# alibaba/easydist

Measured on AMD Instinct MI355X. Metric: gpt2_train_samples_per_sec, higher is better.
Workload: dtype bf16; 1 GPU; model=gpt2-small, global_batch=64, seq_len=1024, parallelism=auto(dp1)

## Files before the change

### easydist_amd/ops/csrc/gemm_kernels.hip

```cpp
#include "common.h"
#include "attn_block_map.h"
#include "gemm_tn_map.h"
#include <torch/extension.h>
#include <ATen/cuda/CUDAContext.h>

using f32x4 = __attribute__((ext_vector_type(4))) float;
using bf16x8v = __attribute__((ext_vector_type(8))) __bf16;
using v4s = __attribute__((ext_vector_type(4))) short;
using v8s = __attribute__((ext_vector_type(8))) short;

DEVINL void glds16(const void* gsrc, void* lds_dst) {
  __builtin_amdgcn_global_load_lds(
      (const __attribute__((address_space(1))) unsigned int*)gsrc,
      (__attribute__((address_space(3))) unsigned int*)lds_dst, 16, 0, 0);
}

DEVINL void raw_barrier() { __builtin_amdgcn_s_barrier(); }

#define GELU_C 0.7978845608028654f
#define GELU_A 0.044715f

DEVINL float fast_tanh(float u) {
  return 1.f - 2.f / (__expf(2.f * u) + 1.f);
}

DEVINL float act_apply(int act, float x, float aux) {
  if (act == 1 || act == 3) {
    float u = GELU_C * (x + GELU_A * x * x * x);
    return 0.5f * x * (1.f + fast_tanh(u));
  }
  if (act == 2 || act == 4) {
    float u = GELU_C * (aux + GELU_A * aux * aux * aux);
    float t = fast_tanh(u);
    float d = 0.5f * (1.f + t)
              + 0.5f * aux * (1.f - t * t) * GELU_C
                    * (1.f + 3.f * GELU_A * aux * aux);
    return x * d;
  }
  if (act >= 5) {
    float u = GELU_C * (x + GELU_A * x * x * x);
    return 0.5f * x * (1.f + fast_tanh(u));
  }
  return x;
}

__global__ void __launch_bounds__(256)
gelu_fwd_kernel(const bf16* __restrict__ X, bf16* __restrict__ Y, long n) {
  long i = ((long)blockIdx.x * blockDim.x + threadIdx.x) * 8;
  for (; i + 7 < n; i += (long)gridDim.x * blockDim.x * 8) {
    bf16x8v x = *reinterpret_cast<const bf16x8v*>(&X[i]);
    bf16x8v y;
    #pragma unroll
    for (int e = 0; e < 8; ++e)
      y[e] = (__bf16)act_apply(1, bf2f((bf16)x[e]), 0.f);
    *reinterpret_cast<bf16x8v*>(&Y[i]) = y;
  }
}

__global__ void __launch_bounds__(256)
gelu_bwd_kernel(const bf16* __restrict__ G, const bf16* __restrict__ X,
                bf16* __restrict__ Y, long n) {
  long i = ((long)blockIdx.x * blockDim.x + threadIdx.x) * 8;
  for (; i + 7 < n; i += (long)gridDim.x * blockDim.x * 8) {
    bf16x8v g = *reinterpret_cast<const bf16x8v*>(&G[i]);
    bf16x8v x = *reinterpret_cast<const bf16x8v*>(&X[i]);
    bf16x8v y;
    #pragma unroll
    for (int e = 0; e < 8; ++e)
      y[e] = (__bf16)act_apply(2, bf2f((bf16)g[e]), bf2f((bf16)x[e]));
    *reinterpret_cast<bf16x8v*>(&Y[i]) = y;
  }
}

#define BM 128
#define BN 128
#define BK 32

extern "C" __global__ void __launch_bounds__(256)
gemm_nt_128(const bf16* __restrict__ A, const bf16* __restrict__ Bt,
            bf16* __restrict__ C, const bf16* __restrict__ bias,
            int M, int N, int K) {
  extern __shared__ __attribute__((aligned(16))) char smem[];
  const unsigned ATILE = BM * BK * 2;
  const unsigned BUF = 2 * ATILE;

  unsigned nwg_m = (M + BM - 1) / BM, nwg_n = (N + BN - 1) / BN;
  unsigned wg = xcd_swizzle(blockIdx.x, nwg_m * nwg_n);
  const unsigned m0 = (wg / nwg_n) * BM;
  const unsigned n0 = (wg % nwg_n) * BN;

  const int t = threadIdx.x;
  const int lane = t % WAVE;
  const int wave = t / WAVE;
  const int wm = (wave / 2) * 64;
  const int wn = (wave % 2) * 64;

  auto stage = [&](int buf, int k0) {
    #pragma unroll
    for (int p = 0; p < 2; ++p) {
      int e = (t + p * 256) * 8;
      int row = e / BK, col = e % BK;
      int grow = min((int)m0 + row, M - 1);
      const bf16* src = A + (long)grow * K + k0 + col;
      glds16(src, smem + buf * BUF + (p * 256 + wave * 64) * 16);
    }
    #pragma unroll
    for (int p = 0; p < 2; ++p) {
      int e = (t + p * 256) * 8;
      int row = e / BK, col = e % BK;
      int grow = min((int)n0 + row, N - 1);
      const bf16* src = Bt + (long)grow * K + k0 + col;
      glds16(src, smem + buf * BUF + ATILE + (p * 256 + wave * 64) * 16);
    }
  };

  f32x4 acc[4][4];
  #pragma unroll
  for (int i = 0; i < 4; ++i)
    #pragma unroll
    for (int j = 0; j < 4; ++j)
      acc[i][j] = {0.f, 0.f, 0.f, 0.f};

  stage(0, 0);
  __builtin_amdgcn_s_waitcnt(0);
  __syncthreads();

  const int frag_row = lane & 15;
  const int frag_k = (lane >> 4) * 8;

  int nk = K / BK;
  for (int kt = 0; kt < nk; ++kt) {
    int buf = kt & 1;
    if (kt + 1 < nk) stage(buf ^ 1, (kt + 1) * BK);
    bf16x8v a_frag[4], b_frag[4];
    const char* base = smem;
    #pragma unroll
    for (int i = 0; i < 4; ++i) {
      unsigned off = buf * BUF + ((wm + i * 16 + frag_row) * BK + frag_k) * 2;
      a_frag[i] = *reinterpret_cast<const bf16x8v*>(base + off);
    }
    #pragma unroll
    for (int j = 0; j < 4; ++j) {
      unsigned off = buf * BUF + ATILE +
                     ((wn + j * 16 + frag_row) * BK + frag_k) * 2;
      b_frag[j] = *reinterpret_cast<const bf16x8v*>(base + off);
    }
    #pragma unroll
    for (int i = 0; i < 4; ++i)
      #pragma unroll
      for (int j = 0; j < 4; ++j)
        acc[i][j] = __builtin_amdgcn_mfma_f32_16x16x32_bf16(
            a_frag[i], b_frag[j], acc[i][j], 0, 0, 0);
    __builtin_amdgcn_s_waitcnt(0);
    __syncthreads();
  }

  const int c_col = lane & 15;
  const int c_row0 = (lane >> 4) * 4;
  float bias_v[4] = {0.f, 0.f, 0.f, 0.f};
  if (bias) {
    #pragma unroll
    for (int j = 0; j < 4; ++j)
      bias_v[j] = bf2f(bias[min((int)(n0 + wn + j * 16 + c_col), N - 1)]);
  }
  #pragma unroll
  for (int i = 0; i < 4; ++i) {
    #pragma unroll
    for (int j = 0; j < 4; ++j) {
      #pragma unroll
      for (int reg = 0; reg < 4; ++reg) {
        int gm = m0 + wm + i * 16 + c_row0 + reg;
        int gn = n0 + wn + j * 16 + c_col;
        if (gm < M && gn < N)
          C[(long)gm * N + gn] = f2bf(acc[i][j][reg] + bias_v[j]);
      }
    }
  }
}

#define BM2 256
#define BN2 256
#define BK2 64
#define HALF_B 16384u
#define BUF_B 65536u

DEVINL unsigned sw32(unsigned x) { return x ^ (((x >> 8) & 7u) << 4); }

extern "C" __global__ void __launch_bounds__(512)
gemm_nt_256(const bf16* __restrict__ A, const bf16* __restrict__ Bt,
            bf16* __restrict__ C, const bf16* __restrict__ bias,
            bf16* __restrict__ aux, int act, int M, int N, int K) {
  extern __shared__ __attribute__((aligned(16))) char smem[];

  unsigned nwg_m = (M + BM2 - 1) / BM2, nwg_n = (N + BN2 - 1) / BN2;
  unsigned wg = xcd_swizzle(blockIdx.x, nwg_m * nwg_n);
  const unsigned m0 = (wg / nwg_n) * BM2;
  const unsigned n0 = (wg % nwg_n) * BN2;

  const int t = threadIdx.x;
  const int lane = t % WAVE;
  const int wave = t / WAVE;
  const int wr = wave >> 2;
  const int wc = wave & 3;

  auto stage_a = [&](int parity, int k0, int h) {
    unsigned dst0 = parity * BUF_B + h * HALF_B;
    #pragma unroll
    for (int i = 0; i < 2; ++i) {
      unsigned p = (i * 512 + t) * 16;
      unsigned L = sw32(p);
      int s = L >> 13;
      int row = (L >> 7) & 63;
      int k = (L & 127) >> 1;
      int grow = min((int)m0 + s * 128 + h * 64 + row, M - 1);
      glds16(A + (long)grow * K + k0 + k,
             smem + dst0 + (i * 512 + wave * 64) * 16);
    }
  };
  auto stage_b = [&](int parity, int k0, int h) {
    unsigned dst0 = parity * BUF_B + 32768u + h * HALF_B;
    #pragma unroll
    for (int i = 0; i < 2; ++i) {
      unsigned p = (i * 512 + t) * 16;
      unsigned L = sw32(p);
      int s = (L >> 12) & 3;
      int col = (L >> 7) & 31;
      int k = (L & 127) >> 1;
      int gcol = min((int)n0 + s * 64 + h * 32 + col, N - 1);
      glds16(Bt + (long)gcol * K + k0 + k,
             smem + dst0 + (i * 512 + wave * 64) * 16);
    }
  };

  const int fr = lane & 15;
  const int fg = lane >> 4;
  auto read_a = [&](bf16x8v (&a)[4][2], int tile, int mh) {
    unsigned base = (tile & 1) * BUF_B + mh * HALF_B;
    #pragma unroll
    for (int i = 0; i < 4; ++i)
      #pragma unroll
      for (int kk = 0; kk < 2; ++kk) {
        unsigned L = wr * 8192u + (i * 16 + fr) * 128u +
                     (kk * 32 + fg * 8) * 2u;
        a[i][kk] = *reinterpret_cast<const bf16x8v*>(smem + base + sw32(L));
      }
  };
  auto read_b = [&](bf16x8v (&b)[2][2], int tile, int nh) {
    unsigned base = (tile & 1) * BUF_B + 32768u + nh * HALF_B;
    #pragma unroll
    for (int j = 0; j < 2; ++j)
      #pragma unroll
      for (int kk = 0; kk < 2; ++kk) {
        unsigned L = wc * 4096u + (j * 16 + fr) * 128u +
                     (kk * 32 + fg * 8) * 2u;
        b[j][kk] = *reinterpret_cast<const bf16x8v*>(smem + base + sw32(L));
      }
  };

  f32x4 acc[8][4];
  #pragma unroll
  for (int i = 0; i < 8; ++i)
    #pragma unroll
    for (int j = 0; j < 4; ++j)
      acc[i][j] = {0.f, 0.f, 0.f, 0.f};

  bf16x8v a_frag[4][2], b_frag[2][2], b0_frag[2][2];
  const int NT = K / BK2;

  auto k_of = [&](int t) { return t < NT ? t * BK2 : 0; };

  stage_a(0, 0, 0); stage_a(0, 0, 1); stage_b(0, 0, 0); stage_b(0, 0, 1);
  stage_a(1, k_of(1), 0); stage_b(1, k_of(1), 1); stage_a(1, k_of(1), 1);
  asm volatile("s_waitcnt vmcnt(6)" ::: "memory");
  raw_barrier();

  auto mfma_quad = [&](int mh, int nh, bf16x8v (&bf)[2][2]) {
    __builtin_amdgcn_s_setprio(1);
    #pragma unroll
    for (int i = 0; i < 4; ++i)
      #pragma unroll
      for (int j = 0; j < 2; ++j)
        #pragma unroll
        for (int kk = 0; kk < 2; ++kk)
          acc[mh * 4 + i][nh * 2 + j] = __builtin_amdgcn_mfma_f32_16x16x32_bf16(
              a_frag[i][kk], bf[j][kk], acc[mh * 4 + i][nh * 2 + j],
              0, 0, 0);
    __builtin_amdgcn_s_setprio(0);
  };

  for (int T = 0; T < NT; ++T) {
    read_a(a_frag, T, 0);
    read_b(b0_frag, T, 0);
    read_b(b_frag, T, 1);
    stage_b((T + 1) & 1, k_of(T + 1), 0);
    mfma_quad(0, 0, b0_frag);
    raw_barrier();
    stage_a(T & 1, k_of(T + 2), 0);
    mfma_quad(0, 1, b_frag);
    raw_barrier();
    read_a(a_frag, T, 1);
    stage_b(T & 1, k_of(T + 2), 1);
    mfma_quad(1, 1, b_frag);
    raw_barrier();
    stage_a(T & 1, k_of(T + 2), 1);
    asm volatile("s_waitcnt vmcnt(6)" ::: "memory");
    mfma_quad(1, 0, b0_frag);
    raw_barrier();
  }

  asm volatile("s_waitcnt vmcnt(0)" ::: "memory");
  raw_barrier();
  bf16* share = reinterpret_cast<bf16*>(smem) + wave * 8192;
  const unsigned wm = wr * 128, wn = wc * 64;
  float bias_v[4] = {0.f, 0.f, 0.f, 0.f};
  if (bias) {
    #pragma unroll
    for (int j = 0; j < 4; ++j)
      bias_v[j] = bf2f(bias[min((int)(n0 + wn + j * 16 + fr), N - 1)]);
  }
  #pragma unroll
  for (int i = 0; i < 8; ++i)
    #pragma unroll
    for (int j = 0; j < 4; ++j)
      #pragma unroll
      for (int r = 0; r < 4; ++r) {
        int row = i * 16 + fg * 4 + r;
        int col = j * 16 + fr;
        share[row * 64 + col] = f2bf(acc[i][j][r] + bias_v[j]);
      }
  lds_fence();
  #pragma unroll
  for (int tt = 0; tt < 16; ++tt) {
    int row = tt * 8 + (lane >> 3);
    int colc = (lane & 7) * 8;
    int gm = m0 + wm + row;
    int gn = n0 + wn + colc;
    if (gm < (int)M && gn + 8 <= (int)N) {
      bf16x8v val = *reinterpret_cast<const bf16x8v*>(&share[row * 64 + colc]);
      if (act) {
        bf16x8v av{};
        if (act == 2 || act == 4)
          av = *reinterpret_cast<const bf16x8v*>(&aux[(long)gm * N + gn]);
        else if (act >= 5)
          *reinterpret_cast<bf16x8v*>(&aux[(long)gm * N + gn]) = val;
        #pragma unroll
        for (int e = 0; e < 8; ++e)
          val[e] = (__bf16)act_apply(act, bf2f((bf16)val[e]),
                                     bf2f((bf16)av[e]));
      }
      *reinterpret_cast<bf16x8v*>(&C[(long)gm * N + gn]) = val;
    } else if (gm < (int)M) {
      for (int e = 0; e < 8 && gn + e < (int)N; ++e) {
        float xv = bf2f(share[row * 64 + colc + e]);
        float axv = (act == 2 || act == 4)
                        ? bf2f(aux[(long)gm * N + gn + e]) : 0.f;
        if (act >= 5) aux[(long)gm * N + gn + e] = f2bf(xv);
        C[(long)gm * N + gn + e] = f2bf(act_apply(act, xv, axv));
      }
    }
  }
}

#define TBR 32
#define TBP 128
#define TBP2 256

constexpr unsigned tn_img_bytes(int tile) { return TBR * tile * 2; }
constexpr unsigned tn_lds_bytes(int tile, int ring) {
  return (ring ? 3 : 2) * 2 * tn_img_bytes(tile);
}

DEVINL int tn_unswz(int pos) { return ((pos >> 2) & 1) | ((pos & 3) << 1); }

template <int NTHR>
DEVINL void tn_stage(const bf16* src, long ld, int r0, int p0, int pmax,
                     char* dst_base, int t, int wave) {
  #pragma unroll
  for (int i = 0; i < 2; ++i) {
    unsigned p = (i * NTHR + t) * 16;
    int chunk16 = p >> 10;
    unsigned w = p & 1023u;
    int bpos = w >> 7;
    int blk = tn_unswz(bpos);
    int rr = blk * 4 + ((w & 127) >> 5);
    int pp = chunk16 * 16 + ((w & 31) >> 1);
    int gp = min(p0 + pp, pmax - 8);
    glds16(src + (long)(r0 + rr) * ld + gp,
           dst_base + (i * NTHR + wave * 64) * 16);
  }
}

DEVINL bf16x8v tn_frag(const char* img, int chunk, int lane) {
  const char* base = img + chunk * 1024 + (lane >> 4) * 128 + (lane & 15) * 8;
  v4s lo = __builtin_amdgcn_ds_read_tr16_b64_v4i16(
      (__attribute__((address_space(3))) v4s*)base);
  v4s hi = __builtin_amdgcn_ds_read_tr16_b64_v4i16(
      (__attribute__((address_space(3))) v4s*)(base + 512));
  v8s out = __builtin_shufflevector(lo, hi, 0, 1, 2, 3, 4, 5, 6, 7);
  return __builtin_bit_cast(bf16x8v, out);
}

template <int TILE, int RING>
DEVINL void tn_body(const bf16* __restrict__ Ag, const bf16* __restrict__ Bg,
                    float* __restrict__ Cw, float* __restrict__ Asum, int R,
                    int P, int Q, int splitr, int map_mode) {
  extern __shared__ __attribute__((aligned(16))) char smem[];
  constexpr int NTHR = 2 * TILE;
  constexpr int NJ = TILE / 32;
  const unsigned IMG = tn_img_bytes(TILE);
  const unsigned BUF = 2 * IMG;

  unsigned nwg_p = (P + TILE - 1) / TILE, nwg_q = (Q + TILE - 1) / TILE;
  unsigned ntile = nwg_p * nwg_q;
  const TnBlock blk = gemm_tn_map(blockIdx.x, ntile, splitr, map_mode);
  const unsigned tile = blk.tile, slice = blk.slice;
  const unsigned p0 = (tile / nwg_q) * TILE;
  const unsigned q0 = (tile % nwg_q) * TILE;

  int nrt_all = R / TBR;
  int per = (nrt_all + splitr - 1) / splitr;
  int rt0 = slice * per;
  int rt1 = min(nrt_all, rt0 + per);
  if (rt0 >= rt1) return;

  const int t = threadIdx.x;
  const int lane = t % WAVE;
  const int wave = t / WAVE;
  const int wp = (wave >> 1) * 64;
  const int wq = (wave & 1) * (TILE / 2);

  auto stage = [&](int buf, int rt) {
    if (rt < rt1) {
      tn_stage<NTHR>(Ag, P, rt * TBR, p0, P, smem + buf * BUF, t, wave);
      tn_stage<NTHR>(Bg, Q, rt * TBR, q0, Q, smem + buf * BUF + IMG, t, wave);
    }
  };

  f32x4 acc[4][NJ];
  float asum_acc[4] = {0.f, 0.f, 0.f, 0.f};
  #pragma unroll
  for (int i = 0; i < 4; ++i)
    #pragma unroll
    for (int j = 0; j < NJ; ++j)
      acc[i][j] = {0.f, 0.f, 0.f, 0.f};

  auto compute = [&](const char* img) {
    bf16x8v a_frag[4], b_frag[NJ];
    #pragma unroll
    for (int i = 0; i < 4; ++i)
      a_frag[i] = tn_frag(img, (wp >> 4) + i, lane);
    if (Asum && q0 == 0 && (wave & 1) == 0) {
      #pragma unroll
      for (int i = 0; i < 4; ++i) {
        float acc_s = 0.f;
        #pragma unroll
        for (int u = 0; u < 8; ++u) acc_s += bf2f((bf16)a_frag[i][u]);
        asum_acc[i] += acc_s;
      }
    }
    #pragma unroll
    for (int j = 0; j < NJ; ++j)
      b_frag[j] = tn_frag(img + IMG, (wq >> 4) + j, lane);
    #pragma unroll
    for (int i = 0; i < 4; ++i)
      #pragma unroll
      for (int j = 0; j < NJ; ++j)
        acc[i][j] = __builtin_amdgcn_mfma_f32_16x16x32_bf16(
            a_frag[i], b_frag[j], acc[i][j], 0, 0, 0);
  };

  if constexpr (RING) {
    stage(0, rt0);
    stage(1, rt0 + 1);
    int buf = 0;
    for (int rt = rt0; rt < rt1; ++rt) {
      if (rt + 1 < rt1)
        asm volatile("s_waitcnt vmcnt(4)" ::: "memory");
      else
        asm volatile("s_waitcnt vmcnt(0)" ::: "memory");
      raw_barrier();
      stage(buf == 0 ? 2 : buf - 1, rt + 2);
      compute(smem + buf * BUF);
      buf = buf == 2 ? 0 : buf + 1;
    }
  } else {
    stage(0, rt0);
    __builtin_amdgcn_s_waitcnt(0);
    __syncthreads();
    for (int rt = rt0; rt < rt1; ++rt) {
      int buf = (rt - rt0) & 1;
      stage(buf ^ 1, rt + 1);
      compute(smem + buf * BUF);
      __builtin_amdgcn_s_waitcnt(0);
      __syncthreads();
    }
  }

  if (Asum && q0 == 0 && (wave & 1) == 0) {
    #pragma unroll
    for (int i = 0; i < 4; ++i) {
      float v = asum_acc[i];
      v += __shfl_down(v, 32, WAVE);
      v += __shfl_down(v, 16, WAVE);
      if (lane < 16) {
        int gp = p0 + wp + i * 16 + lane;
        if (gp < P) atomicAdd(&Asum[gp], v);
      }
    }
  }
  const int c_col = lane & 15;
  const int c_row0 = (lane >> 4) * 4;
  #pragma unroll
  for (int i = 0; i < 4; ++i)
    #pragma unroll
    for (int j = 0; j < NJ; ++j)
      #pragma unroll
      for (int reg = 0; reg < 4; ++reg) {
        int gp = p0 + wp + i * 16 + c_row0 + reg;
        int gq = q0 + wq + j * 16 + c_col;
        if (gp < P && gq < Q) {
          if (splitr == 1)
            Cw[(long)gp * Q + gq] = acc[i][j][reg];
          else
            atomicAdd(&Cw[(long)gp * Q + gq], acc[i][j][reg]);
        }
      }
}

#define TN_KERNEL(name, tile, ring)                                         \
  extern "C" __global__ void __launch_bounds__(2 * tile)                    \
  name(const bf16* __restrict__ Ag, const bf16* __restrict__ Bg,            \
       float* __restrict__ Cw, float* __restrict__ Asum, int R, int P,      \
       int Q, int splitr, int map_mode) {                                   \
    tn_body<tile, ring>(Ag, Bg, Cw, Asum, R, P, Q, splitr, map_mode);       \
  }
TN_KERNEL(gemm_tn_kernel, TBP, 0)
TN_KERNEL(gemm_tn_256_kernel, TBP2, 1)
TN_KERNEL(gemm_tn_256_drain_kernel, TBP2, 0)


at::Tensor gemm_nt_act(const at::Tensor& a, const at::Tensor& bt,
                       const std::optional<at::Tensor>& bias, int64_t act,
                       const std::optional<at::Tensor>& aux) {
  TORCH_CHECK(a.dtype() == at::kBFloat16 && bt.dtype() == at::kBFloat16);
  TORCH_CHECK(a.is_contiguous() && bt.is_contiguous(),
              "gemm_nt wants K-contiguous operands");
  const long M = a.size(0), K = a.size(1), N = bt.size(0);
  TORCH_CHECK(bt.size(1) == K);
  TORCH_CHECK(K % BK == 0, "gemm_nt: K must be a multiple of 32");
  TORCH_CHECK(N % 8 == 0, "gemm_nt: N must be a multiple of 8");
  auto c = at::empty({M, N}, a.options());
  auto stream = at::cuda::getCurrentCUDAStream();
  const bf16* bias_p = bias ? (const bf16*)bias->data_ptr() : nullptr;
  TORCH_CHECK(!(act == 2 || act >= 4) || aux,
              "gemm_nt: activation modes 2/4/5/6 need aux");
  if (K % BK2 == 0 && M >= BM2 && N >= 128) {
    unsigned nwg = ((M + BM2 - 1) / BM2) * ((N + BN2 - 1) / BN2);
    bf16* aux_p = aux ? (bf16*)aux->data_ptr() : nullptr;
    hipLaunchKernelGGL(gemm_nt_256, dim3(nwg), dim3(512), 2 * BUF_B, stream,
        (const bf16*)a.data_ptr(), (const bf16*)bt.data_ptr(),
        (bf16*)c.data_ptr(), bias_p, aux_p, (int)act, (int)M, (int)N,
        (int)K);
  } else {
    unsigned nwg = ((M + BM - 1) / BM) * ((N + BN - 1) / BN);
    size_t lds = 2 * 2 * BM * BK * 2;
    hipLaunchKernelGGL(gemm_nt_128, dim3(nwg), dim3(256), lds, stream,
        (const bf16*)a.data_ptr(), (const bf16*)bt.data_ptr(),
        (bf16*)c.data_ptr(), bias_p, (int)M, (int)N, (int)K);
    if (act) {
      if (act == 1) c = at::gelu(c, "tanh");
      else if (act == 3) c = at::gelu(c);
      else if (act == 2) c = at::gelu_backward(c, aux.value(), "tanh");
      else if (act == 4) c = at::gelu_backward(c, aux.value(), "none");
      else if (act >= 5) {
        aux.value().copy_(c);
        c = at::gelu(c, "tanh");
      }
    }
  }
  return c;
}

at::Tensor gemm_nt(const at::Tensor& a, const at::Tensor& bt,
                   const std::optional<at::Tensor>& bias) {
  return gemm_nt_act(a, bt, bias, 0, std::nullopt);
}

at::Tensor gelu_fast(const at::Tensor& x) {
  TORCH_CHECK(x.dtype() == at::kBFloat16 && x.is_contiguous());
  const long n = x.numel();
  TORCH_CHECK(n % 8 == 0, "gelu_fast: numel multiple of 8");
  auto y = at::empty_like(x);
  long thr = n / 8;
  unsigned grid = (unsigned)std::min<long>((thr + 255) / 256, 8192);
  auto stream = at::cuda::getCurrentCUDAStream();
  hipLaunchKernelGGL(gelu_fwd_kernel, dim3(grid), dim3(256), 0, stream,
                     (const bf16*)x.data_ptr(), (bf16*)y.data_ptr(), n);
  return y;
}

at::Tensor gelu_bwd_fast(const at::Tensor& g, const at::Tensor& x) {
  TORCH_CHECK(g.dtype() == at::kBFloat16 && g.is_contiguous());
  TORCH_CHECK(x.dtype() == at::kBFloat16 && x.is_contiguous());
  const long n = x.numel();
  TORCH_CHECK(g.numel() == n && n % 8 == 0);
  auto y = at::empty_like(x);
  long thr = n / 8;
  unsigned grid = (unsigned)std::min<long>((thr + 255) / 256, 8192);
  auto stream = at::cuda::getCurrentCUDAStream();
  hipLaunchKernelGGL(gelu_bwd_kernel, dim3(grid), dim3(256), 0, stream,
                     (const bf16*)g.data_ptr(), (const bf16*)x.data_ptr(),
                     (bf16*)y.data_ptr(), n);
  return y;
}

std::tuple<at::Tensor, at::Tensor>
gemm_nt_gelu(const at::Tensor& a, const at::Tensor& bt,
             const std::optional<at::Tensor>& bias, bool tanh_approx) {
  const long M = a.size(0), K = a.size(1), N = bt.size(0);
  if (K % BK2 == 0 && M >= BM2 && N >= 128) {
    auto pre = at::empty({M, N}, a.options());
    auto act = gemm_nt_act(a, bt, bias, tanh_approx ? 5 : 6, pre);
    return {act, pre};
  }
  auto pre = gemm_nt_act(a, bt, bias, 0, std::nullopt);
  auto act = at::gelu(pre, tanh_approx ? "tanh" : "none");
  return {act, pre};
}

std::tuple<at::Tensor, at::Tensor> gemm_tn_asum(const at::Tensor& a,
                                                const at::Tensor& b);

static inline int ed_tn_map_mode() {
  const char* e = getenv("EASYDIST_TN_MAP");
  return (e && atoi(e) == 0) ? TN_MAP_TILE_MAJOR : TN_MAP_SLICE_MAJOR;
}

static at::Tensor tn_launch(const at::Tensor& a, const at::Tensor& b,
                            float* asum_p) {
  const int map_mode = ed_tn_map_mode();
  TORCH_CHECK(a.dtype() == at::kBFloat16 && b.dtype() == at::kBFloat16);
  TORCH_CHECK(a.is_contiguous() && b.is_contiguous());
  const long R = a.size(0), P = a.size(1), Q = b.size(0) == R ? b.size(1) : -1;
  TORCH_CHECK(Q > 0, "gemm_tn: reduce dims must match");
  TORCH_CHECK(R % TBR == 0, "gemm_tn: R must be a multiple of 32");
  TORCH_CHECK(P % TBP == 0 && Q % TBP == 0,
              "gemm_tn: P, Q must be multiples of 128");
  bool big = R / TBR >= 64 && P >= TBP2 && Q >= TBP2;
  unsigned ntile;
  int splitr = 1;
  if (big) {
    ntile = ((P + TBP2 - 1) / TBP2) * ((Q + TBP2 - 1) / TBP2);
    const int target = 256;
    splitr = std::max(1, target / (int)ntile);
    if (const char* e = getenv("EASYDIST_TN256_SPLITR"))
      if (atoi(e) > 0) splitr = atoi(e);
    splitr = std::min((long)splitr, R / TBR / 8);
    splitr = std::max(1, std::min(splitr, 64));
  } else {
    ntile = (P / TBP) * (Q / TBP);
    while (ntile * splitr < 512 && splitr < 16 &&
           (R / TBR) % (splitr * 2) == 0 && (R / TBR) / (splitr * 2) >= 1)
      splitr *= 2;
  }
  auto cw = splitr == 1
      ? at::empty({P, Q}, a.options().dtype(at::kFloat))
      : at::zeros({P, Q}, a.options().dtype(at::kFloat));
  auto stream = at::cuda::getCurrentCUDAStream();
  if (big) {
    const char* se = getenv("EASYDIST_TN256_STAGING");
    const bool ring = !(se && atoi(se) == 0);
    auto kern = ring ? gemm_tn_256_kernel : gemm_tn_256_drain_kernel;
    size_t lds = tn_lds_bytes(TBP2, ring);
    hipLaunchKernelGGL(kern, dim3(ntile * splitr), dim3(2 * TBP2),
        lds, stream,
        (const bf16*)a.data_ptr(), (const bf16*)b.data_ptr(),
        cw.data_ptr<float>(), asum_p, (int)R, (int)P, (int)Q, splitr,
        map_mode);
  } else {
    size_t lds = tn_lds_bytes(TBP, 0);
    hipLaunchKernelGGL(gemm_tn_kernel, dim3(ntile * splitr), dim3(2 * TBP),
        lds, stream,
        (const bf16*)a.data_ptr(), (const bf16*)b.data_ptr(),
        cw.data_ptr<float>(), asum_p, (int)R, (int)P, (int)Q, splitr,
        map_mode);
  }
  return cw;
}

at::Tensor gemm_tn(const at::Tensor& a, const at::Tensor& b) {
  return tn_launch(a, b, nullptr).to(at::kBFloat16);
}

std::tuple<at::Tensor, at::Tensor> gemm_tn_asum(const at::Tensor& a,
                                                const at::Tensor& b) {
  auto asum = at::zeros({a.size(1)}, a.options().dtype(at::kFloat));
  auto cw = tn_launch(a, b, asum.data_ptr<float>());
  return {cw.to(at::kBFloat16), asum};
}
```

Before: 794.9 samples/sec.

## Fuse split-R TN GEMM epilogue with persistent workspace and bf16 sweep

Reworks how the weight-gradient TN GEMM finishes. By default it keeps a persistent per-stream fp32 workspace that the split-R kernel accumulates into atomically. A small sweep kernel then converts it to bf16, copies out the bias sum and re-zeroes the workspace, replacing the per-call zeros allocation and separate .to(bf16) cast. A store mode with per-slice slabs and a last-arriving-block reduction is also added, and single-slice cases now write bf16 directly through an LDS bounce. This adds workspace state keyed by stream and counter logic, and falls back to the old path during graph capture.

```diff
diff --git a/easydist_amd/ops/csrc/gemm_kernels.hip b/easydist_amd/ops/csrc/gemm_kernels.hip
--- a/easydist_amd/ops/csrc/gemm_kernels.hip
+++ b/easydist_amd/ops/csrc/gemm_kernels.hip
@@ -3,6 +3,9 @@
 #include "gemm_tn_map.h"
 #include <torch/extension.h>
 #include <ATen/cuda/CUDAContext.h>
+#include <map>
+#include <mutex>
+#include <type_traits>
 
 using f32x4 = __attribute__((ext_vector_type(4))) float;
 using bf16x8v = __attribute__((ext_vector_type(8))) __bf16;
@@ -366,8 +369,13 @@
 #define TBP2 256
 
 constexpr unsigned tn_img_bytes(int tile) { return TBR * tile * 2; }
+constexpr int tn_bounce_ld(int tile) { return tile / 2 + 4; }
+constexpr unsigned tn_bounce_bytes(int tile) {
+  return (tile / 32) * 16 * tn_bounce_ld(tile) * 4;
+}
 constexpr unsigned tn_lds_bytes(int tile, int ring) {
-  return (ring ? 3 : 2) * 2 * tn_img_bytes(tile);
+  unsigned stage = (ring ? 3 : 2) * 2 * tn_img_bytes(tile);
+  return stage > tn_bounce_bytes(tile) ? stage : tn_bounce_bytes(tile);
 }
 
 DEVINL int tn_unswz(int pos) { return ((pos >> 2) & 1) | ((pos & 3) << 1); }
@@ -390,6 +398,12 @@
   }
 }
 
+#define TN_FIN_LEGACY 0
+#define TN_FIN_STORE 1
+#define TN_FIN_SWEEP 2
+
+struct alignas(8) bf16x4 { bf16 v[4]; };
+
 DEVINL bf16x8v tn_frag(const char* img, int chunk, int lane) {
   const char* base = img + chunk * 1024 + (lane >> 4) * 128 + (lane & 15) * 8;
   v4s lo = __builtin_amdgcn_ds_read_tr16_b64_v4i16(
@@ -402,8 +416,9 @@
 
 template <int TILE, int RING>
 DEVINL void tn_body(const bf16* __restrict__ Ag, const bf16* __restrict__ Bg,
-                    float* __restrict__ Cw, float* __restrict__ Asum, int R,
-                    int P, int Q, int splitr, int map_mode) {
+                    float* Cw, bf16* __restrict__ Cout, float* Asum,
+                    float* AsumP, int* cnt, int R, int P, int Q, int splitr,
+                    int map_mode, int finish) {
   extern __shared__ __attribute__((aligned(16))) char smem[];
   constexpr int NTHR = 2 * TILE;
   constexpr int NJ = TILE / 32;
@@ -422,6 +437,8 @@
   int rt0 = slice * per;
   int rt1 = min(nrt_all, rt0 + per);
   if (rt0 >= rt1) return;
+  const int nslice = (nrt_all + per - 1) / per;
+  const bool single = nslice == 1;
 
   const int t = threadIdx.x;
   const int lane = t % WAVE;
@@ -504,35 +521,157 @@
       v += __shfl_down(v, 16, WAVE);
       if (lane < 16) {
         int gp = p0 + wp + i * 16 + lane;
-        if (gp < P) atomicAdd(&Asum[gp], v);
+        if (gp < P) {
+          if (finish == TN_FIN_LEGACY) atomicAdd(&Asum[gp], v);
+          else if (single) Asum[gp] = v;
+          else AsumP[(long)slice * P + gp] = v;
+        }
       }
     }
   }
   const int c_col = lane & 15;
   const int c_row0 = (lane >> 4) * 4;
-  #pragma unroll
-  for (int i = 0; i < 4; ++i)
-    #pragma unroll
-    for (int j = 0; j < NJ; ++j)
-      #pragma unroll
-      for (int reg = 0; reg < 4; ++reg) {
-        int gp = p0 + wp + i * 16 + c_row0 + reg;
-        int gq = q0 + wq + j * 16 + c_col;
+  const long PQ = (long)P * Q;
+  if (finish == TN_FIN_LEGACY) {
+    #pragma unroll
+    for (int i = 0; i < 4; ++i)
+      #pragma unroll
+      for (int j = 0; j < NJ; ++j)
+        #pragma unroll
+        for (int reg = 0; reg < 4; ++reg) {
+          int gp = p0 + wp + i * 16 + c_row0 + reg;
+          int gq = q0 + wq + j * 16 + c_col;
+          if (gp < P && gq < Q) {
+            if (splitr == 1)
+              Cw[(long)gp * Q + gq] = acc[i][j][reg];
+            else
+              atomicAdd(&Cw[(long)gp * Q + gq], acc[i][j][reg]);
+          }
+        }
+    return;
+  }
+  {
+    constexpr int LDW = tn_bounce_ld(TILE);
+    constexpr int LPR = TILE / 8;
+    __syncthreads();
+    float* share = reinterpret_cast<float*>(smem) + wave * 16 * LDW;
+    float* slab = Cw + (long)slice * PQ;
+    const int b_row = lane / LPR, b_col = (lane % LPR) * 4;
+    #pragma unroll
+    for (int i = 0; i < 4; ++i) {
+      #pragma unroll
+      for (int j = 0; j < NJ; ++j)
+        #pragma unroll
+        for (int reg = 0; reg < 4; ++reg)
+          share[(c_row0 + reg) * LDW + j * 16 + c_col] = acc[i][j][reg];
+      lds_fence();
+      #pragma unroll
+      for (int k = 0; k < 16 * LPR / WAVE; ++k) {
+        int row = k * (WAVE / LPR) + b_row;
+        f32x4 v = *reinterpret_cast<const f32x4*>(&share[row * LDW + b_col]);
+        int gp = p0 + wp + i * 16 + row;
+        int gq = q0 + wq + b_col;
         if (gp < P && gq < Q) {
-          if (splitr == 1)
-            Cw[(long)gp * Q + gq] = acc[i][j][reg];
-          else
-            atomicAdd(&Cw[(long)gp * Q + gq], acc[i][j][reg]);
+          if (single) {
+            bf16x4 o;
+            #pragma unroll
+            for (int e = 0; e < 4; ++e) o.v[e] = f2bf(v[e]);
+            *reinterpret_cast<bf16x4*>(&Cout[(long)gp * Q + gq]) = o;
+          } else {
+            *reinterpret_cast<f32x4*>(&slab[(long)gp * Q + gq]) = v;
+          }
         }
       }
+      lds_fence();
+    }
+  }
+  if (single) return;
+
+  __builtin_amdgcn_fence(__ATOMIC_RELEASE, "agent");
+  asm volatile("s_waitcnt vmcnt(0)" ::: "memory");
+  __syncthreads();
+  volatile int* ticket = reinterpret_cast<volatile int*>(smem);
+  if (t == 0)
+    *ticket = __hip_atomic_fetch_add(&cnt[tile], 1, __ATOMIC_RELAXED,
+                                     __HIP_MEMORY_SCOPE_AGENT);
+  __syncthreads();
+  if (*ticket != nslice - 1) return;
+  __builtin_amdgcn_fence(__ATOMIC_ACQUIRE, "agent");
+  asm volatile("s_waitcnt vmcnt(0)" ::: "memory");
+  if (t == 0)
+    __hip_atomic_store(&cnt[tile], 0, __ATOMIC_RELAXED,
+                       __HIP_MEMORY_SCOPE_AGENT);
+
+  if (Asum && q0 == 0 && t < TILE && (int)p0 + t < P) {
+    float s = 0.f;
+    for (int sl = 0; sl < nslice; ++sl) s += AsumP[(long)sl * P + p0 + t];
+    Asum[p0 + t] = s;
+  }
+  constexpr int TPR = TILE / 4;
+  constexpr int RPP = NTHR / TPR;
+  const int f_col = q0 + (t % TPR) * 4;
+  const bool q_ok = f_col < Q;
+  const int l_col = min(f_col, Q - 4);
+  auto reduce = [&](auto nr_c, auto ns_c) {
+    constexpr int NR = decltype(nr_c)::value, NS = decltype(ns_c)::value;
+    for (int rb = t / TPR; rb < TILE; rb += NR * RPP) {
+      f32x4 s[NR];
+      #pragma unroll
+      for (int u = 0; u < NR; ++u) s[u] = {0.f, 0.f, 0.f, 0.f};
+      #pragma unroll NS
+      for (int sl = 0; sl < nslice; ++sl)
+        #pragma unroll
+        for (int u = 0; u < NR; ++u) {
+          long off = (long)min((int)p0 + rb + u * RPP, P - 1) * Q + l_col;
+          s[u] += *reinterpret_cast<const f32x4*>(&Cw[sl * PQ + off]);
+        }
+      #pragma unroll
+      for (int u = 0; u < NR; ++u) {
+        int gp = p0 + rb + u * RPP;
+        if (gp < P && q_ok) {
+          bf16x4 o;
+          #pragma unroll
+          for (int e = 0; e < 4; ++e) o.v[e] = f2bf(s[u][e]);
+          *reinterpret_cast<bf16x4*>(&Cout[(long)gp * Q + f_col]) = o;
+        }
+      }
+    }
+  };
+  using std::integral_constant;
+  if constexpr (TILE == TBP2)
+    reduce(integral_constant<int, 4>{}, integral_constant<int, 8>{});
+  else
+    reduce(integral_constant<int, 2>{}, integral_constant<int, 2>{});
+}
+
+__global__ void __launch_bounds__(256)
+tn_sweep_kernel(float* __restrict__ ws, bf16* __restrict__ C,
+                     float* __restrict__ asum, long PQ, int P) {
+  const long stride = (long)gridDim.x * blockDim.x;
+  const long i0 = (long)blockIdx.x * blockDim.x + threadIdx.x;
+  const f32x4 zero = {0.f, 0.f, 0.f, 0.f};
+  for (long i = i0; i < PQ / 4; i += stride) {
+    f32x4 v = reinterpret_cast<const f32x4*>(ws)[i];
+    bf16x4 o;
+    #pragma unroll
+    for (int e = 0; e < 4; ++e) o.v[e] = f2bf(v[e]);
+    reinterpret_cast<bf16x4*>(C)[i] = o;
+    reinterpret_cast<f32x4*>(ws)[i] = zero;
+  }
+  if (asum)
+    for (long i = i0; i < P; i += stride) {
+      asum[i] = ws[PQ + i];
+      ws[PQ + i] = 0.f;
+    }
 }
 
 #define TN_KERNEL(name, tile, ring)                                         \
   extern "C" __global__ void __launch_bounds__(2 * tile)                    \
-  name(const bf16* __restrict__ Ag, const bf16* __restrict__ Bg,            \
-       float* __restrict__ Cw, float* __restrict__ Asum, int R, int P,      \
-       int Q, int splitr, int map_mode) {                                   \
-    tn_body<tile, ring>(Ag, Bg, Cw, Asum, R, P, Q, splitr, map_mode);       \
+  name(const bf16* __restrict__ Ag, const bf16* __restrict__ Bg, float* Cw, \
+       bf16* __restrict__ Cout, float* Asum, float* AsumP, int* cnt, int R, \
+       int P, int Q, int splitr, int map_mode, int finish) {                \
+    tn_body<tile, ring>(Ag, Bg, Cw, Cout, Asum, AsumP, cnt, R, P, Q,        \
+                        splitr, map_mode, finish);                          \
   }
 TN_KERNEL(gemm_tn_kernel, TBP, 0)
 TN_KERNEL(gemm_tn_256_kernel, TBP2, 1)
@@ -636,8 +775,45 @@
   return (e && atoi(e) == 0) ? TN_MAP_TILE_MAJOR : TN_MAP_SLICE_MAJOR;
 }
 
+static inline int ed_tn_finish() {
+  const char* e = getenv("EASYDIST_TN_FINISH");
+  if (!e) return TN_FIN_SWEEP;
+  const int v = atoi(e);
+  return v == 0 ? TN_FIN_LEGACY : v == 1 ? TN_FIN_STORE : TN_FIN_SWEEP;
+}
+
+struct TnState { at::Tensor cnt, ws; };
+
+static bool tn_state(const at::Tensor& like, hipStream_t stream, long ntile,
+                     long ws_elems, int** cnt_p, float** ws_p) {
+  static std::mutex mu;
+  static auto* states =
+      new std::map<std::pair<int, hipStream_t>, TnState>();
+  std::lock_guard<std::mutex> guard(mu);
+  TnState& st = (*states)[{(int)like.get_device(), stream}];
+  const bool grow_cnt = !st.cnt.defined() || st.cnt.numel() < ntile;
+  const bool grow_ws =
+      ws_elems > 0 && (!st.ws.defined() || st.ws.numel() < ws_elems);
+  if (grow_cnt || grow_ws) {
+    hipStreamCaptureStatus cap = hipStreamCaptureStatusNone;
+    if (hipStreamIsCapturing(stream, &cap) != hipSuccess) {
+      (void)hipGetLastError();
+      return false;
+    }
+    if (cap != hipStreamCaptureStatusNone) return false;
+    if (grow_cnt)
+      st.cnt = at::zeros({std::max(ntile, 1024L)},
+                         like.options().dtype(at::kInt));
+    if (grow_ws)
+      st.ws = at::zeros({ws_elems}, like.options().dtype(at::kFloat));
+  }
+  *cnt_p = st.cnt.data_ptr<int>();
+  *ws_p = ws_elems > 0 ? st.ws.data_ptr<float>() : nullptr;
+  return true;
+}
+
 static at::Tensor tn_launch(const at::Tensor& a, const at::Tensor& b,
-                            float* asum_p) {
+                            at::Tensor* asum_out) {
   const int map_mode = ed_tn_map_mode();
   TORCH_CHECK(a.dtype() == at::kBFloat16 && b.dtype() == at::kBFloat16);
   TORCH_CHECK(a.is_contiguous() && b.is_contiguous());
@@ -663,38 +839,76 @@
            (R / TBR) % (splitr * 2) == 0 && (R / TBR) / (splitr * 2) >= 1)
       splitr *= 2;
   }
-  auto cw = splitr == 1
-      ? at::empty({P, Q}, a.options().dtype(at::kFloat))
-      : at::zeros({P, Q}, a.options().dtype(at::kFloat));
+  const long per = (R / TBR + splitr - 1) / splitr;
+  const long nslice = (R / TBR + per - 1) / per;
   auto stream = at::cuda::getCurrentCUDAStream();
+  const auto f32 = a.options().dtype(at::kFloat);
+
+  int finish = ed_tn_finish();
+  int* cnt_p = nullptr;
+  float* cw_p = nullptr;
+  const long ws_elems = finish == TN_FIN_SWEEP ? P * Q + P : 0;
+  if (finish != TN_FIN_LEGACY && nslice > 1 &&
+      !tn_state(a, stream, ntile, ws_elems, &cnt_p, &cw_p))
+    finish = TN_FIN_LEGACY;
+  const bool sweep = finish == TN_FIN_SWEEP && nslice > 1;
+  int kfinish = finish;
+  if (finish == TN_FIN_SWEEP) kfinish = sweep ? TN_FIN_LEGACY : TN_FIN_STORE;
+
+  at::Tensor cw, c, asum, asum_part;
+  float* asum_p = nullptr;
+  if (finish == TN_FIN_LEGACY) {
+    cw = splitr == 1 ? at::empty({P, Q}, f32) : at::zeros({P, Q}, f32);
+    cw_p = cw.data_ptr<float>();
+    if (asum_out) asum = at::zeros({P}, f32);
+  } else {
+    c = at::empty({P, Q}, a.options());
+    if (asum_out) asum = at::empty({P}, f32);
+    if (nslice > 1 && !sweep) {
+      if (finish == TN_FIN_STORE) {
+        cw = at::empty({nslice, P, Q}, f32);
+        cw_p = cw.data_ptr<float>();
+      }
+      if (asum_out) asum_part = at::empty({nslice, P}, f32);
+    }
+  }
+  if (asum_out) asum_p = sweep ? cw_p + P * Q : asum.data_ptr<float>();
+  const bf16* a_p = (const bf16*)a.data_ptr();
+  const bf16* b_p = (const bf16*)b.data_ptr();
+  bf16* c_p = c.defined() ? (bf16*)c.data_ptr() : nullptr;
+  float* part_p = asum_part.defined() ? asum_part.data_ptr<float>() : nullptr;
   if (big) {
     const char* se = getenv("EASYDIST_TN256_STAGING");
     const bool ring = !(se && atoi(se) == 0);
     auto kern = ring ? gemm_tn_256_kernel : gemm_tn_256_drain_kernel;
     size_t lds = tn_lds_bytes(TBP2, ring);
     hipLaunchKernelGGL(kern, dim3(ntile * splitr), dim3(2 * TBP2),
-        lds, stream,
-        (const bf16*)a.data_ptr(), (const bf16*)b.data_ptr(),
-        cw.data_ptr<float>(), asum_p, (int)R, (int)P, (int)Q, splitr,
-        map_mode);
+        lds, stream, a_p, b_p, cw_p, c_p, asum_p, part_p, cnt_p, (int)R,
+        (int)P, (int)Q, splitr, map_mode, kfinish);
   } else {
     size_t lds = tn_lds_bytes(TBP, 0);
     hipLaunchKernelGGL(gemm_tn_kernel, dim3(ntile * splitr), dim3(2 * TBP),
-        lds, stream,
-        (const bf16*)a.data_ptr(), (const bf16*)b.data_ptr(),
-        cw.data_ptr<float>(), asum_p, (int)R, (int)P, (int)Q, splitr,
-        map_mode);
-  }
-  return cw;
+        lds, stream, a_p, b_p, cw_p, c_p, asum_p, part_p, cnt_p, (int)R,
+        (int)P, (int)Q, splitr, map_mode, kfinish);
+  }
+  if (sweep) {
+    const long n4 = P * Q / 4;
+    unsigned grid = (unsigned)std::min<long>((n4 + 255) / 256, 2048);
+    hipLaunchKernelGGL(tn_sweep_kernel, dim3(grid), dim3(256), 0, stream,
+        cw_p, c_p, asum_out ? asum.data_ptr<float>() : nullptr, P * Q,
+        (int)P);
+  }
+  if (asum_out) *asum_out = asum;
+  return finish == TN_FIN_LEGACY ? cw.to(at::kBFloat16) : c;
 }
 
 at::Tensor gemm_tn(const at::Tensor& a, const at::Tensor& b) {
-  return tn_launch(a, b, nullptr).to(at::kBFloat16);
+  return tn_launch(a, b, nullptr);
 }
 
 std::tuple<at::Tensor, at::Tensor> gemm_tn_asum(const at::Tensor& a,
                                                 const at::Tensor& b) {
-  auto asum = at::zeros({a.size(1)}, a.options().dtype(at::kFloat));
-  auto cw = tn_launch(a, b, asum.data_ptr<float>());
-  return {cw.to(at::kBFloat16), asum};
-}
+  at::Tensor asum;
+  auto c = tn_launch(a, b, &asum);
+  return {c, asum};
+}
```

Result: no change. 794.9 samples/sec (-0.0%).
